# pinellolab/CRISPResso2

Measured on NVIDIA H100. Metric: reads/sec aligned+classified (250 bp, single amplicon), higher is better.
Workload: dtype int32

## Files before the change

crispresso2_b200/_lib.py:

```python
import ctypes as C
import os

import numpy as np

_HERE = os.path.dirname(os.path.abspath(__file__))
DEFAULT_LIB = os.path.join(_HERE, "libc2b200.so")

MAX_Q = 8
MAX_SEEDS = 8
MAX_READ_LEN = 512
MAX_REF_LEN = 1024
MAX_REFS = 32

F_IGNORE_SUBSTITUTIONS = 1
F_IGNORE_INSERTIONS = 2
F_IGNORE_DELETIONS = 4
F_EXPAND_AMBIGUOUS = 8
F_ASSIGN_FIRST = 16
F_DISCARD_INDEL_READS = 32
F_NO_STRAND_SEARCH = 64
F_NO_PAIRING = 128
F_HDR_REF1 = 256
F_NO_RING = 512
F_LEGACY_INS = 1024
# ... 37 lines not shown
                ("n_seeds", C.c_int32), ("tot_exon_len_mod", C.c_int32), ("coding_mask", C.c_void_p)]


ALN_DTYPE = np.dtype([("n_match", "<u2"), ("aln_len", "<u2"), ("score_milli", "<i4"), ("strand", "u1"),
                      ("status", "u1"), ("n_edits", "<u2"), ("insertion_n", "<u2"), ("deletion_n", "<u2"),
                      ("substitution_n", "<u2"), ("n_ins_all", "<u2"), ("n_ins_win", "<u2"), ("n_del_all", "<u2"),
                      ("n_del_win", "<u2"), ("n_del_pos_all", "<u2"), ("n_sub_all", "<u2"),
                      ("irregular_ends", "u1"), ("modified", "u1")])
REC_DTYPE = np.dtype([("winner_mask", "<u4"), ("best_score_milli", "<i4"), ("best_ref", "<i2"), ("n_winners", "u1"),
                      ("ambiguous", "u1"), ("status", "<u4")])
EDIT_DTYPE = np.dtype([("a", "<u2"), ("b", "<u2"), ("type", "u1"), ("in_window", "u1"), ("base", "u1"), ("pad", "u1")])
assert ALN_DTYPE.itemsize == 32 and REC_DTYPE.itemsize == 16 and EDIT_DTYPE.itemsize == 8

EXPORTS = ["c2b_create", "c2b_destroy", "c2b_last_error", "c2b_configure", "c2b_set_edit_cap", "c2b_string_width", "c2b_align_batch",
           "c2b_align_batch_compact", "c2b_ops_words", "c2b_expand_alignment", "c2b_expand_batch", "c2b_ops_device",
           "c2b_align_batch_device", "c2b_set_pair_order", "c2b_sync", "c2b_stream", "c2b_last_kernel_ms", "c2b_launch_count", "c2b_path_counts", "c2b_band_reruns", "c2b_ring_counts", "c2b_diag_counts", "c2b_route_counts", "c2b_diag_popcount_reads",
           "c2b_counts_layout", "c2b_counts_hist_layout", "c2b_counts_reset", "c2b_counts_read", "c2b_counts_device", "c2b_global_align",
           "c2b_classify_aligned", "c2b_classify_aligned_flags", "c2b_host_alloc", "c2b_host_free",
           "c2b_fastq_dedup", "c2b_fastq_dedup_buffer", "c2b_fastq_gpu_available", "c2b_fastq_dedup_gpu", "c2b_fastq_dedup_gpu_buffer", "c2b_sam_dedup_gpu_buffer", "c2b_sam_dedup_buffer", "c2b_fastq_n_reads", "c2b_fastq_n_unique", "c2b_fastq_max_len",
           "c2b_fastq_seqs", "c2b_fastq_offsets", "c2b_fastq_counts", "c2b_fastq_first_index", "c2b_fastq_free",
           "c2b_fastq_last_error", "c2b_fastq_filter", "c2b_fastq_filter_pair", "c2b_rc_merge_weights", "c2b_screen_reads", "c2b_serial_stats",
           "c2b_consensus_from_pairs", "c2b_alleles_build", "c2b_alleles_free", "c2b_alleles_n", "c2b_alleles_order", "c2b_alleles_arena", "c2b_alleles_offsets",
           "c2b_alleles_lengths", "c2b_alleles_write_tsv", "c2b_alleles_around_cut", "c2b_alleles_cut_width", "c2b_alleles_cut_fetch",
           "c2b_annotate_build", "c2b_annotate_free", "c2b_annotate_n", "c2b_annotate_arena", "c2b_annotate_offsets",
           "c2b_annotate_cigar_arena", "c2b_annotate_cigar_offsets", "c2b_annotate_flags", "c2b_annotate_mapq", "c2b_annotate_first",
           "c2b_annotate_last_record", "c2b_annotate_record_arena", "c2b_annotate_record_offsets", "c2b_annotate_write_fastq",
           "c2b_annotate_write_sam", "c2b_annotate_write_sam_passthrough"]

_cache = {}


# ... 46 lines not shown
    L.c2b_last_kernel_ms.argtypes = [vp]
    L.c2b_launch_count.restype = i64
    L.c2b_launch_count.argtypes = [vp]
    L.c2b_path_counts.restype = C.c_int
    L.c2b_path_counts.argtypes = [vp, C.POINTER(i64), C.POINTER(i64)]
    L.c2b_band_reruns.restype = i64
    L.c2b_band_reruns.argtypes = [vp]
    L.c2b_ring_counts.restype = C.c_int
    L.c2b_ring_counts.argtypes = [vp, C.POINTER(i64), C.POINTER(i64)]
    L.c2b_diag_counts.restype = C.c_int
    L.c2b_diag_counts.argtypes = [vp, C.POINTER(i64), C.POINTER(i64), C.POINTER(i64)]
    L.c2b_route_counts.restype = C.c_int
    L.c2b_route_counts.argtypes = [vp, C.POINTER(i64), C.POINTER(i64)]
    L.c2b_diag_popcount_reads.restype = C.c_int
    L.c2b_diag_popcount_reads.argtypes = [vp, C.POINTER(i64)]
    L.c2b_counts_layout.restype = C.c_int
    L.c2b_counts_layout.argtypes = [vp, C.POINTER(i32), C.POINTER(i32), C.POINTER(i32), C.POINTER(i32)]
    L.c2b_counts_hist_layout.restype = C.c_int
    L.c2b_counts_hist_layout.argtypes = [vp, C.POINTER(i32), C.POINTER(i32), C.POINTER(i32)]
    L.c2b_counts_reset.restype = C.c_int
    L.c2b_counts_reset.argtypes = [vp]
    L.c2b_counts_read.restype = C.c_int
    L.c2b_counts_read.argtypes = [vp, vp, C.c_size_t]
    L.c2b_counts_device.restype = C.c_int
    L.c2b_counts_device.argtypes = [vp, C.POINTER(vp), C.POINTER(C.c_size_t)]
    L.c2b_global_align.restype = C.c_int
    L.c2b_global_align.argtypes = [vp, C.c_char_p, i32, C.c_char_p, i32, C.c_char_p, i32, vp, vp, i32, i32,
                                   C.c_char_p, C.c_char_p, C.POINTER(i32), C.POINTER(i32)]
    L.c2b_classify_aligned.restype = C.c_int
    L.c2b_classify_aligned.argtypes = [vp, C.c_char_p, C.c_char_p, i32, C.c_char_p, i32, vp, i32, vp, vp]
# ... 84 lines not shown
```

crispresso2_b200/csrc/c2b_core.cuh:

```cuda
#pragma once
#include <stdint.h>
#include "c2b200.h"

#ifndef C2B_EMU
#include <cuda_runtime.h>
#define C2B_DEV __device__ __forceinline__
#define C2B_DEVNOINL __device__ __noinline__
namespace wp {
C2B_DEV int lane() { return threadIdx.x & 31; }
C2B_DEV int shfl_up(int v, int d) { return __shfl_up_sync(0xffffffffu, v, d); }
C2B_DEV int shfl(int v, int src) { return __shfl_sync(0xffffffffu, v, src); }
C2B_DEV uint32_t shflu(uint32_t v, int src) { return __shfl_sync(0xffffffffu, v, src); }
C2B_DEV uint32_t shflu_up(uint32_t v, int d) { return __shfl_up_sync(0xffffffffu, v, d); }
C2B_DEV int shfl_xor(int v, int m) { return __shfl_xor_sync(0xffffffffu, v, m); }
C2B_DEV uint32_t ballot(bool p) { return __ballot_sync(0xffffffffu, p); }
C2B_DEV void sync() { __syncwarp(); }
#ifdef C2B_X_INLINE_BARRIER
C2B_DEV
#else
__device__ __noinline__
#endif
void grp_sync(int g)
{
    const int w = (int)(threadIdx.x >> 5), sh = 31 - __clz(g);
// ... 72 lines not shown
    uint32_t pk_XB, pk_YB, pk_M00;
    const uint32_t *prof2;
    const uint32_t *cIe2;
    const uint32_t *g42;
    int32_t rg_ok, rg_smax, rg_gmax, rg_gsum;
    int32_t dg_ok, dg_S, dg_thr4;
    int32_t dg_c4[2 * 4 + 1];
    int32_t dg_two, dg_a4, dg_b4;
    int32_t rt_ok, rt_thr;
    int32_t rt_mx;
    int32_t rt_c[32];
    const uint4 *rt_pl;
};
constexpr int32_t RT_OFF = -(1 << 30);
constexpr int RN_DLO = 17, RN_DHI = 11;

struct WorkBlock {
    unsigned long long pair_items, single_items, band_reruns, ring_kept, ring_sent, align_settled;
    unsigned long long diag_proved, diag_listed, tier2, routed, kept;
    unsigned long long diag_popc;
    struct Launch {
        unsigned long long align_next, tier2_next, general_next;
        unsigned long long widest;
        unsigned long long left_n, tier2_n, narrow_n, diag_n;
    } launch;
};
constexpr size_t WORK_BYTES = 32 * 8;
static_assert(sizeof(WorkBlock) <= WORK_BYTES, "work block");

struct KParams {
    const uint8_t *reads; const int64_t *offsets; int64_t n_reads;
    const int32_t *count, *qweight, *ref_id;
    const int32_t *pair_order;
    c2b_read_rec *recs; c2b_aln_rec *alns; uint8_t *strings; c2b_edit *edits;
    int32_t W, edit_cap;
    const RefDev *refs; int32_t n_refs;
    int32_t out_refs, ops_refs;
    int32_t go, ge, seed_count, seed_min; uint32_t flags; int32_t nq;
    uint8_t alpha[C2B_MAX_Q]; uint8_t comp[C2B_MAX_Q];
    uint32_t *tb; int64_t tb_words_per_warp; int32_t TS;
    uint32_t *tbb; int64_t tbb_words_per_warp;
    uint32_t *tbq;
    int32_t *bnd; int64_t bnd_words_per_warp;
    uint64_t *opsbuf;
    uint64_t *rgops;
    WorkBlock *wb;
    unsigned long long *work_counter;
    uint64_t *gops; uint32_t *gmeta; int32_t NW;
    int32_t *left;
    int32_t *left2;
    int32_t *left0;
    int32_t *left1;
    int32_t route;
    const unsigned long long *n_dev;
    int32_t vstride, hstride;
    const uint32_t *stage_src;
    int32_t stage_bytes;
    const uint8_t *lut;
    int32_t phase_sync;
    const uint64_t *forced_ops;
    const int32_t *forced_n;
};

C2B_DEV int64_t oslot(const KParams &P, int64_t rd, int r) { return rd * P.out_refs + (P.ref_id ? 0 : r); }
C2B_DEV int64_t nreads(const KParams &P) { return P.n_dev ? (int64_t)*P.n_dev : P.n_reads; }

C2B_DEV const RefDev &refdev(const KParams &P, int r) { return P.refs[r]; }

// ... 1448 lines not shown
```

crispresso2_b200/csrc/c2b_engine.cu:

```cuda
#include <algorithm>
#include <atomic>
#include <mutex>
#ifndef C2B_EMU
#include <sched.h>
#include <sys/syscall.h>
#include <unistd.h>
#include <cctype>
#endif
#include <chrono>
#include <cstdio>
#include <cstdlib>
#include <cstring>
#include <string>
#include <thread>
#include <vector>

#include "c2b_core.cuh"
#include "c2b_split.cuh"
#include "c2b_annotate.cuh"
#include "c2b_fastq_int.h"

using namespace c2b;

#ifndef C2B_EMU
// ... 762 lines not shown
    const size_t tile = (size_t)e->prm.nq * e->prm.nq * r0.Ipad * 4;
    const bool can_stage = r0.pk_maxJ > 0 && !e->forced_ops;
    auto add = [&](StepKind kind, const KParams &K, int grid, int block, size_t smem) { plan.step[plan.n++] = Step{kind, K, grid, block, smem}; };
    if (split) {
        KParams A = P;
        A.left = b.left;
        if (can_stage && tile <= (size_t)e->stage_cap_a) { A.stage_bytes = (int32_t)tile; A.stage_src = r0.prof2; }
        const size_t smem_a = sizeof(ASmem) * WARPS_PER_CTA + 128 + (size_t)A.stage_bytes;
        const bool narrow = b.left2 && !P.pair_order && plan.one && !sw.no_narrow;
        if (narrow) A.left2 = b.left2;
        const bool diag = narrow && b.left0 && e->diag_any && b.n_reads >= 16 && !sw.no_diag;
        const bool route = diag && b.left1 && !sw.no_route;
        if (diag) {
            KParams D = P;
            D.left0 = b.left0;
            if (route) { D.left1 = b.left1; D.left2 = b.left2; D.route = sw.route_all ? 2 : 1; }
            const int64_t units = (b.n_reads + 31) / 32;
            add(STEP_DIAG, D, (int)std::min<int64_t>((units + D_WARPS_PER_CTA - 1) / D_WARPS_PER_CTA, (int64_t)e->grid_a * 16), D_WARPS_PER_CTA * 32, 0);
            A.pair_order = route ? b.left1 : b.left0; A.n_dev = route ? &wb->launch.narrow_n : &wb->launch.diag_n;
        }
        add(STEP_ALIGN, A, e->grid_a, WARPS_PER_CTA * 32, smem_a);
        if (narrow) {
            KParams A2 = A;
            A2.left2 = nullptr;
            A2.pair_order = b.left2; A2.n_dev = &wb->launch.tier2_n; A2.work_counter = &wb->launch.tier2_next;
            add(STEP_ALIGN, A2, e->grid_a, WARPS_PER_CTA * 32, smem_a);
        }
        KParams B = P;
        B.pair_order = diag ? b.left0 : nullptr; B.n_dev = diag ? &wb->launch.diag_n : nullptr;
        add(STEP_CLASSIFY, B, e->grid_b, B_WARPS_PER_CTA * 32, 0);
// ... 84 lines not shown
    RTCHK(rt_zero(&((WorkBlock *)e->work.p)->launch, sizeof(WorkBlock::Launch), cs));
    if (b.gmeta) RTCHK(rt_zero(b.gmeta, (size_t)b.n_reads * (b.ref_id ? 1 : e->n_refs) * 4, cs));
    if ((rc = run_plan(e, plan, cs))) return rc;
    e->launches += plan.n;
    return C2B_OK;
}

static int ensure_ops(c2b_engine *e, DevBuf &gops, DevBuf &gmeta, DevBuf &left, DevBuf &left2, DevBuf &left0, DevBuf &left1, int64_t n_reads,
                      int nr, int W)
{
    int rc;
    if ((rc = ensure(e, gops, (size_t)n_reads * nr * (W / 32) * 8))) return rc;
    if ((rc = ensure(e, gmeta, (size_t)n_reads * nr * 4))) return rc;
    if ((rc = ensure(e, left, (size_t)(n_reads + 8) * 4))) return rc;
    if ((rc = ensure(e, left2, (size_t)(n_reads + 16) * 4))) return rc;
    if ((rc = ensure(e, left0, (size_t)(n_reads + 16) * 4))) return rc;
    if ((rc = ensure(e, left1, (size_t)(n_reads + 16) * 4))) return rc;
    return C2B_OK;
}

int c2b_align_batch_device(c2b_engine *e, const uint8_t *d_reads, const int64_t *d_offsets, int64_t n_reads,
                           int32_t max_read_len, const int32_t *d_count, const int32_t *d_qweight,
                           const int32_t *d_ref_id, c2b_read_rec *d_recs, c2b_aln_rec *d_alns,
                           uint8_t *d_strings, c2b_edit *d_edits)
{
    if (!e || !e->configured) return fail(e, C2B_E_STATE, "c2b_align_batch_device: engine not configured");
#ifndef C2B_EMU
    cudaSetDevice(e->device);
#endif
    if (max_read_len < 1) max_read_len = 1;
    const int W = (e->max_I + max_read_len + 31) & ~31, nr = d_ref_id ? 1 : e->n_refs;
// ... 70 lines not shown
    if (proved) *proved = (int64_t)v.diag_proved;
    if (tier1) *tier1 = (int64_t)v.diag_listed;
    if (tier2) *tier2 = (int64_t)v.tier2;
    return C2B_OK;
}

int c2b_diag_popcount_reads(c2b_engine *e, int64_t *reads)
{
    if (!e || !e->work.p) return fail(e, C2B_E_STATE, "c2b_diag_popcount_reads: nothing launched yet");
    WorkBlock v;
    RTCHK(rt_d2h(&v, e->work.p, sizeof v, e->stream));
    RTCHK(rt_sync(e->stream));
    if (reads) *reads = (int64_t)v.diag_popc;
    return C2B_OK;
}

int c2b_route_counts(c2b_engine *e, int64_t *routed, int64_t *kept)
{
    if (!e || !e->work.p) return fail(e, C2B_E_STATE, "c2b_route_counts: nothing launched yet");
    WorkBlock v;
    RTCHK(rt_d2h(&v, e->work.p, sizeof v, e->stream));
    RTCHK(rt_sync(e->stream));
    if (routed) *routed = (int64_t)v.routed;
    if (kept) *kept = (int64_t)v.kept;
    return C2B_OK;
}

int c2b_ring_counts(c2b_engine *e, int64_t *ring_pairs, int64_t *ring_fallbacks)
{
    if (!e) return C2B_E_ARG;
// ... 616 lines not shown
```

crispresso2_b200/csrc/c2b_split.cuh:

```cuda
#pragma once
#include "c2b_core.cuh"

namespace c2b {

constexpr uint32_t GM_NONE = 0, GM_ALIGNED = 1;

C2B_DEV uint32_t gmeta_pack(int n, int strand, uint32_t state) { return (uint32_t)n | ((uint32_t)strand << 16) | (state << 24); }

struct ASmem {
    uint8_t fw[2][RG_COMBO], rc[2][RG_COMBO];
    uint8_t combo[8][RG_COMBO];
    uint32_t fin[96];
    uint8_t lut[256];
};

C2B_DEV void asmem_init(const KParams &P, ASmem &S)
{
    const int lane = wp::lane();
    for (int k = lane; k < 256; k += 32) S.lut[k] = P.lut[k];
    wp::sync();
}

C2B_DEV int64_t read_at(const KParams &P, int64_t idx) { return P.pair_order ? (int64_t)P.pair_order[idx] : idx; }

// ... 15 lines not shown
    const int lane = wp::lane();
    bool bad = false;
    for (int base = 0; base < J; base += 128) {
        uint8_t ch[4];
#pragma unroll
        for (int e = 0; e < 4; e++) { const int p = base + lane + 32 * e; ch[e] = p < J ? src[p] : (uint8_t)P.alpha[0]; }
#pragma unroll
        for (int e = 0; e < 4; e++) {
            const int p = base + lane + 32 * e;
            int code = lut[ch[e]];
            if (code == 255) { bad = true; code = 0; }
            if (p < J) { fw[p] = (uint8_t)code; rc[J - 1 - p] = P.comp[code]; }
        }
    }
    return wp::ballot(bad) != 0;
}

template <int RL = 8, int NP = 4>
C2B_DEV void walk_ring4(const KParams &P, const RefDev &R, const int *Jq, const uint2 *__restrict__ tb2, const int *s0, uint32_t mask,
                        Walked *out, const int q0 = 0)
{
    constexpr int NS = 9 * RL, B = 4 * RL;
    const int lane = wp::lane();
    const int hl = lane & 15, hb = lane & 16;
    const int TS = P.TS;
    int i[NP], j[NP], s[NP], n[NP], err[NP];
    uint32_t acc[NP], lo[NP], hi[NP];
#pragma unroll
    for (int q = 0; q < NP; q++) {
        const bool on = (mask >> q) & 1u;
// ... 92 lines not shown
            if (op == OP_NONE) continue;
            if (op == OP_M && (uint32_t)P.alpha[codes[j - 1]] == (uint32_t)R.asc[i - 1]) match++;
            i -= (op != OP_I); j -= (op != OP_J);
        }
        base_i -= tot >> 16; base_j -= tot & 0xffff;
    }
#pragma unroll
    for (int d = 8; d >= 1; d >>= 1) match += wp::shfl_xor(match, d);
    return match;
}

C2B_DEV void align_group(const KParams &P, ASmem &S, const uint32_t *staged_prof, int64_t wq, int warp_slot)
{
    const int lane = wp::lane(), g = lane >> 3;
    const int64_t first = 4 * wq;
    const bool multi = P.ref_id == nullptr && P.n_refs > 1;
    bool quad = (P.tbq != nullptr || P.tb != nullptr) && 2 * first + 7 < nreads(P) && (!multi || P.n_refs <= RG_MAX_REFS);
    int r0 = 0;
    uint32_t ringmask = 0;
    if (quad) {
        const int x = lane & 7;
        const int64_t rd = read_at(P, 2 * first + x);
        const int Jx = (int)(P.offsets[rd + 1] - P.offsets[rd]);
        const int rx = P.ref_id ? P.ref_id[rd] : 0;
        r0 = wp::shfl(rx, 0);
        const int Jn = wp::shfl_xor(Jx, 1);
        bool ok = rx == r0 && Jx == Jn && Jx >= 1 && Jx <= RG_COMBO && Jx + 32 <= P.TS;
        const int k0 = multi ? 0 : r0, k1 = multi ? P.n_refs : r0 + 1;
        for (int k = k0; k < k1; k++) {
            const RefDev &R = refdev(P, k);
            ok = ok && !R.coding && Jx <= R.pk_maxJ;
            const bool rk = P.tbq != nullptr && R.rg_ok && R.I + Jx <= PK_MAX_ALN && Jx - R.I <= RG_MAXD && R.I - Jx <= RG_MAXD;
            if (wp::ballot(rk) == 0xffffffffu) ringmask |= 1u << (k - k0);
        }
        quad = wp::ballot(ok) == 0xffffffffu;
        if (!P.tb && ringmask != (k1 - k0 >= 32 ? 0xffffffffu : (1u << (k1 - k0)) - 1u)) quad = false;
    }
    if (!quad) {
#pragma unroll 1
        for (int q = 0; q < 4; q++) {
            if (2 * (first + q) >= nreads(P)) break;
            const int64_t rdA = read_at(P, 2 * (first + q));
            if (2 * (first + q) + 1 < nreads(P)) leftover_pair(P, rdA, read_at(P, 2 * (first + q) + 1));
            else leftover_one(P, rdA);
        }
        return;
    }
    const int k0 = multi ? 0 : r0, k1 = multi ? P.n_refs : r0 + 1;
    uint2 *tbq = P.tbq ? reinterpret_cast<uint2 *>(P.tbq + (int64_t)warp_slot * P.TS * 64) : nullptr;
    uint32_t okmask = 0, modes = 0;
    uint32_t both2[RG_MAX_REFS] = {0, 0, 0, 0};
    int Jg = 0, Jmax = 0;
#pragma unroll 1
    for (int q = 0; q < 4; q++) {
        const int64_t rdA = read_at(P, 2 * (first + q)), rdB = read_at(P, 2 * (first + q) + 1);
        const int J = (int)(P.offsets[rdA + 1] - P.offsets[rdA]);
        bool bad = false;
#pragma unroll 1
        for (int x = 0; x < 2; x++) bad |= load_codes_a(P, S.lut, P.reads + P.offsets[x ? rdB : rdA], J, S.fw[x], S.rc[x]);
        wp::sync();
        int mAB = 0; bool agree = true;
        uint32_t bothq[RG_MAX_REFS] = {0, 0, 0, 0};
#pragma unroll 1
        for (int k = k0; k < k1; k++) {
            int m = 0;
#pragma unroll 1
            for (int x = 0; x < 2; x++) m |= strand_mode(P, refdev(P, k), S.fw[x], J) << (2 * x);
            if (k == k0) mAB = m;
#pragma unroll
            for (int x = 0; x < 2; x++) {
                const int mk = (m >> (2 * x)) & 3, m0 = (mAB >> (2 * x)) & 3;
                if (mk == 2) bothq[(k - k0) & (RG_MAX_REFS - 1)] |= 1u << x;
                else if (mk != (m0 == 2 ? 0 : m0)) agree = false;
            }
        }
        const int mA = mAB & 3, mB = mAB >> 2;
        if (!bad && agree) {
            const uint8_t *cA = mA == 1 ? S.rc[0] : S.fw[0], *cB = mB == 1 ? S.rc[1] : S.fw[1];
            for (int p = lane; p < J; p += 32) S.combo[q][p] = (uint8_t)(cA[p] * P.nq + cB[p]);
            okmask |= 1u << q; modes |= (uint32_t)mAB << (4 * q);
#pragma unroll
            for (int kk = 0; kk < RG_MAX_REFS; kk++) both2[kk] |= bothq[kk] << (2 * q);
            if (g == q) Jg = J;
            if (J > Jmax) Jmax = J;
        }
        wp::sync();
    }
    uint32_t good2 = 0;
#pragma unroll
    for (int q = 0; q < 4; q++) if ((okmask >> q) & 1u) good2 |= 3u << (2 * q);
    if (!P.tb) {
#pragma unroll
        for (int kk = 0; kk < RG_MAX_REFS; kk++) { good2 &= ~both2[kk]; both2[kk] = 0; }
    }
    int npass = 0, ntried = 0, nboth = 0;
#pragma unroll 1
    for (int k = k0; k < k1 && good2; k++) {
        const RefDev &R = refdev(P, k);
        const uint32_t bothk = both2[(k - k0) & (RG_MAX_REFS - 1)];
        const uint32_t ring2 = good2 & ~bothk;
        nboth += wp::popc(bothk & good2);
        const bool staged = (k == 0 && staged_prof != nullptr);
        uint32_t pass2 = 0;
        if (((ringmask >> (k - k0)) & 1u) && ring2) {
        if (staged) dp_ring<true>(P, R, staged_prof, S.combo[g], Jg, Jmax + R.lstar, tbq, S.fin);
        else dp_ring<false>(P, R, R.prof2, S.combo[g], Jg, Jmax + R.lstar, tbq, S.fin);
        wp::sync();
        const int fl = 3 * ((lane & 24) | (R.lstar & 7));
        const uint32_t cM = Jg > 0 ? S.fin[fl] : PK_SENT, cX = Jg > 0 ? S.fin[fl + 1] : PK_SENT, cY = Jg > 0 ? S.fin[fl + 2] : PK_SENT;
        wp::sync();
        const uint32_t z = wp::max3_2(cM, cY, cX);
        const uint32_t s2 = z & PK_TM;
        const int thr = ring_bound(P, R, Jg) + 512 - P.ge * (R.I + Jg);
        const bool passA = Jg > 0 && (int)((z & 0xffffu) >> 2) > thr, passB = Jg > 0 && (int)(z >> 18) > thr;
        const uint32_t bA = wp::ballot(passA), bB = wp::ballot(passB);
#pragma unroll
        for (int q = 0; q < 4; q++) pass2 |= (((bA >> (8 * q)) & 1u) | (((bB >> (8 * q)) & 1u) << 1)) << (2 * q);
        pass2 &= ring2;
        ntried += wp::popc(ring2);
        {
            int Jq[4], s0[4];
            Walked wk4[4];
            uint32_t walkmask = 0;
#pragma unroll
            for (int q = 0; q < 4; q++) {
                const uint32_t sq = wp::shflu(s2, 8 * q);
                Jq[q] = wp::shfl(Jg, 8 * q);
                s0[q] = (lane & 16) ? (int)(sq >> 16) : (int)(sq & 3u);
                if ((pass2 >> (2 * q)) & 3u) walkmask |= 1u << q;
            }
            walk_ring4(P, R, Jq, tbq, s0, walkmask, wk4);
#pragma unroll
            for (int q = 0; q < 4; q++) {
                if (!((walkmask >> q) & 1u)) continue;
                const Walked &wk = wk4[q];
                const uint32_t eb = wp::ballot(wk.err != 0);
                if (eb & 0xffffu) pass2 &= ~(1u << (2 * q));
                if (eb >> 16) pass2 &= ~(2u << (2 * q));
                const int h = lane >> 4, hl = lane & 15;
                if (!((pass2 >> (2 * q + h)) & 1u)) continue;
                const int64_t rd = read_at(P, 2 * (first + q) + h);
                const int64_t slot = oslot(P, rd, k);
                if (hl < P.NW) P.gops[slot * P.NW + hl] = wk.ops;
                if (hl == 0) {
                    const int mode = (int)((modes >> (4 * q + 2 * h)) & 3u);
                    P.gmeta[slot] = gmeta_pack(wk.n, mode == 1, GM_NONE);
                }
            }
        }
        npass += wp::popc(pass2);
        } else ntried += wp::popc(ring2);
        const uint32_t failed = ring2 & ~pass2;
        if ((failed | (bothk & good2)) && P.tb) {
            uint2 *tb2 = reinterpret_cast<uint2 *>(P.tb + (int64_t)warp_slot * P.tb_words_per_warp);
            int32_t *bnd = P.bnd + (int64_t)warp_slot * P.bnd_words_per_warp;
            const int h = lane >> 4, hl = lane & 15;
#pragma unroll 1
            for (int job = 0; job < 16; job++) {
                const int q = job >> 2, kind = job & 3;
                if (kind == 3) continue;
                const uint32_t fq = (failed >> (2 * q)) & 3u;
                const uint32_t bq = ((bothk & good2) >> (2 * q)) & 3u;
                if (kind == 0 ? fq == 0 : !((bq >> (kind - 1)) & 1u)) continue;
                const int Jp = wp::shfl(Jg, 8 * q);
                const uint8_t *combo = S.combo[q];
                wp::sync();
                if (kind) {
// ... 26 lines not shown
                    const uint32_t bit = 1u << (2 * q + kind - 1);
                    if (eb) good2 &= ~bit;
                    else if (h == pick) {
                        const int64_t rd = read_at(P, 2 * (first + q) + (kind - 1));
                        const int64_t slot = oslot(P, rd, k);
                        if (hl < P.NW) P.gops[slot * P.NW + hl] = wk.ops;
                        if (hl + 16 < P.NW) P.gops[slot * P.NW + 16 + hl] = wk.ops2;
                        if (hl == 0) P.gmeta[slot] = gmeta_pack(wk.n, pick, GM_NONE);
                    }
                }
            }
        }
        pass2 |= bothk & good2;
        good2 &= pass2;
        wp::sync();
    }
#ifndef C2B_EMU
    if (tbq && ringmask) {
        const char *base = reinterpret_cast<const char *>(tbq);
        const int64_t bytes = (int64_t)P.TS * 64 * 4;
        for (int64_t o = (int64_t)lane * 128; o < bytes; o += 32 * 128)
            asm volatile("discard.global.L2 [%0], 128;" ::"l"(base + o) : "memory");
    }
#endif
    if (lane == 0) {
        wp::addg(&P.wb->align_settled, wp::popc(good2));
        wp::addg(&P.wb->ring_kept, npass);
        wp::addg(&P.wb->ring_sent, ntried - npass + nboth + 2 * (k1 - k0) * (4 - wp::popc(okmask)));
    }
#pragma unroll 1
    for (int q = 0; q < 4; q++) {
        const int64_t rdA = read_at(P, 2 * (first + q)), rdB = read_at(P, 2 * (first + q) + 1);
        const uint32_t gq = (good2 >> (2 * q)) & 3u;
        if (gq) {
            const int64_t rd = (lane & 1) ? rdB : rdA;
            const int k = k0 + (lane >> 1);
            if (k < k1 && ((gq >> (lane & 1)) & 1u)) { const int64_t slot = oslot(P, rd, k); P.gmeta[slot] = (P.gmeta[slot] & 0x00ffffffu) | (GM_ALIGNED << 24); }
        }
        if (gq == 0) leftover_pair(P, rdA, rdB);
        else if (gq != 3u) leftover_one(P, gq == 1u ? rdB : rdA);
    }
}

C2B_DEV bool align_narrow16(const KParams &P, ASmem &S, const uint32_t *staged_prof, int64_t w16, int warp_slot)
{
    constexpr int RL = 4, DLO = 4 * RL + 1, DHI = 9 * RL - 4 * RL - 9;
    static_assert(DLO == RN_DLO && DHI == RN_DHI, "the diagonal tier's routing test assumes this band");
    const int lane = wp::lane(), g = lane >> 2;
    const int64_t first = 16 * w16;
    if (!P.left2 || P.tbq == nullptr || first + 15 >= nreads(P) || (P.ref_id == nullptr && P.n_refs > 1)) return false;
    int r0, J0;
    {
        const int64_t rd = read_at(P, first + (lane & 15));
        const int Jx = (int)(P.offsets[rd + 1] - P.offsets[rd]);
        const int rx = P.ref_id ? P.ref_id[rd] : 0;
        r0 = wp::shfl(rx, 0); J0 = wp::shfl(Jx, 0);
        const RefDev &R = refdev(P, r0);
        const bool ok = rx == r0 && Jx == J0 && Jx >= 1 && Jx <= RG_COMBO && Jx + 32 <= P.TS && R.rg_ok && !R.coding && Jx <= R.pk_maxJ &&
                        R.I + Jx <= PK_MAX_ALN && Jx - R.I <= RG_MAXD && R.I - Jx <= RG_MAXD;
        if (wp::ballot(ok) != 0xffffffffu) return false;
    }
    const RefDev &R = refdev(P, r0);
    const int J = J0;
    uint2 *tbq = reinterpret_cast<uint2 *>(P.tbq + (int64_t)warp_slot * P.TS * 64);
    uint32_t modes = 0, use2 = 0;
#pragma unroll 1
    for (int q = 0; q < 8; q++) {
        const int64_t rdA = read_at(P, first + 2 * q), rdB = read_at(P, first + 2 * q + 1);
        bool badA = load_codes_a(P, S.lut, P.reads + P.offsets[rdA], J, S.fw[0], S.rc[0]);
        bool badB = load_codes_a(P, S.lut, P.reads + P.offsets[rdB], J, S.fw[1], S.rc[1]);
        wp::sync();
        int m = 0;
#pragma unroll 1
        for (int x = 0; x < 2; x++) m |= strand_mode(P, R, S.fw[x], J) << (2 * x);
        const int mA = m & 3, mB = m >> 2;
        const uint8_t *cA = mA == 1 ? S.rc[0] : S.fw[0], *cB = mB == 1 ? S.rc[1] : S.fw[1];
        for (int p = lane; p < J; p += 32) S.combo[q][p] = (uint8_t)(cA[p] * P.nq + cB[p]);
        modes |= (uint32_t)m << (4 * q);
        if (!badA && mA != 2) use2 |= 1u << (2 * q);
        if (!badB && mB != 2) use2 |= 2u << (2 * q);
        wp::sync();
    }
    const bool staged = (r0 == 0 && staged_prof != nullptr);
    if (staged) dp_ring<true, RL>(P, R, staged_prof, S.combo[g], J, J + R.lstar, tbq, S.fin);
    else dp_ring<false, RL>(P, R, R.prof2, S.combo[g], J, J + R.lstar, tbq, S.fin);
    wp::sync();
    const int fl = 3 * ((lane & ~(RL - 1)) | (R.lstar & (RL - 1)));
    const uint32_t cM = S.fin[fl], cX = S.fin[fl + 1], cY = S.fin[fl + 2];
    wp::sync();
    const uint32_t z = wp::max3_2(cM, cY, cX);
    const uint32_t s2 = z & PK_TM;
    const int thr = ring_bound(P, R, J, DLO, DHI) + 512 - P.ge * (R.I + J);
    const uint32_t bA = wp::ballot((int)((z & 0xffffu) >> 2) > thr), bB = wp::ballot((int)(z >> 18) > thr);
    uint32_t pass2 = 0;
#pragma unroll
    for (int q = 0; q < 8; q++) pass2 |= (((bA >> (RL * q)) & 1u) | (((bB >> (RL * q)) & 1u) << 1)) << (2 * q);
    pass2 &= use2;
#pragma unroll 1
    for (int half = 0; half < 2; half++) {
        const int q0 = 4 * half;
        int Jq[4], s0[4];
        Walked wk4[4];
        uint32_t walkmask = 0;
#pragma unroll
        for (int q = 0; q < 4; q++) {
            const uint32_t sq = wp::shflu(s2, RL * (q0 + q));
            Jq[q] = J;
            s0[q] = (lane & 16) ? (int)(sq >> 16) : (int)(sq & 3u);
            if ((pass2 >> (2 * (q0 + q))) & 3u) walkmask |= 1u << q;
        }
        if (!walkmask) continue;
        walk_ring4<RL, 4>(P, R, Jq, tbq, s0, walkmask, wk4, q0);
#pragma unroll
        for (int q = 0; q < 4; q++) {
            if (!((walkmask >> q) & 1u)) continue;
            const int qq = q0 + q;
            const Walked &wk = wk4[q];
            const uint32_t eb = wp::ballot(wk.err != 0);
            if (eb & 0xffffu) pass2 &= ~(1u << (2 * qq));
            if (eb >> 16) pass2 &= ~(2u << (2 * qq));
            const int h = lane >> 4, hl = lane & 15;
            if (!((pass2 >> (2 * qq + h)) & 1u)) continue;
            const int64_t rd = read_at(P, first + 2 * qq + h);
            const int64_t slot = oslot(P, rd, r0);
            if (hl < P.NW) P.gops[slot * P.NW + hl] = wk.ops;
            if (hl == 0) P.gmeta[slot] = gmeta_pack(wk.n, (int)((modes >> (4 * qq + 2 * h)) & 3u) == 1, GM_ALIGNED);
        }
    }
#ifndef C2B_EMU
    {
        const char *base = reinterpret_cast<const char *>(tbq);
        const int64_t bytes = (int64_t)P.TS * 64 * 4;
        for (int64_t o = (int64_t)lane * 128; o < bytes; o += 32 * 128)
            asm volatile("discard.global.L2 [%0], 128;" ::"l"(base + o) : "memory");
    }
#endif
    const uint32_t rest = 0xffffu & ~pass2;
    if (lane < 16 && ((rest >> lane) & 1u)) {
        const unsigned long long pos = wp::fetch_add(&P.wb->launch.tier2_n, 1ull);
        P.left2[pos] = (int32_t)read_at(P, first + lane);
    }
    if (lane == 0) {
        wp::addg(&P.wb->align_settled, wp::popc(pass2));
        wp::addg(&P.wb->ring_kept, wp::popc(pass2));
        wp::addg(&P.wb->tier2, 16 - wp::popc(pass2));
    }
    return true;
}

C2B_DEV void align_loop(const KParams &P, ASmem &S, const uint32_t *staged_prof, int warp)
{
    const int lane = wp::lane();
    asmem_init(P, S);
    const int64_t nrd = nreads(P);
    const unsigned ahead = (unsigned)wp::grid_warps();
    if (P.left2) {
        const unsigned total = (unsigned)((nrd + 15) / 16);
        for (;;) {
            unsigned w = 0;
            if (lane == 0) w = (unsigned)wp::fetch_work(P.work_counter);
            w = (unsigned)wp::shfl((int)w, 0);
// ... 569 lines not shown
    }
    sc_flush(acc, P);
}

constexpr int DG_PROVED = 0, DG_KEEP = 1, DG_ROUTE = 2;
struct DSmem {
    uint4 pl[2][10];
    uint8_t raw[2][RG_COMBO + 32];
    int32_t pl_ref;
    uint8_t fw[RG_COMBO], rc[RG_COMBO];
    uint8_t lut[256];
    int64_t off[33];
    int64_t total_bytes;
    int32_t ref[32], cnt[32], qw[32];
    int32_t npop;
};

C2B_DEV uint32_t pl_match(uint4 a, uint4 b) { return ~((a.x ^ b.x) | (a.y ^ b.y)) & a.z & b.z; }
C2B_DEV uint4 pl_shifted(uint4 lo, uint4 hi, int t)
{
    return make_uint4(wp::funnel_r(lo.x, hi.x, t), wp::funnel_r(lo.y, hi.y, t), wp::funnel_r(lo.z, hi.z, t), 0u);
}
C2B_DEV uint32_t pl_below(int n) { return n >= 32 ? ~0u : n <= 0 ? 0u : (1u << n) - 1u; }

C2B_DEV void diag_classify(const KParams &P, const DSmem &S, const RefDev &R, const uint8_t *c, int64_t rd, int r, int strand,
                           long long cnt, long long w, ScAcc<1> &A, bool planes)
{
    const int lane = wp::lane(), I = R.I;
    const uint32_t lt = (1u << lane) - 1u;
    const int64_t slot = oslot(P, rd, r);
// ... 127 lines not shown
    const int pa = 32 * w0 + 2 * lane + 1;
    cand(pa, F0 + incl - e1);
    cand(pa + 1, F0 + incl);
    if (lane == 0) cand(32 * w0, F0);
#pragma unroll
    for (int d = 16; d >= 1; d >>= 1) { const int o = wp::shfl_xor(e, d); if (o > e) e = o; }
    return e > R.rt_thr ? DG_KEEP : DG_ROUTE;
}

C2B_DEV int diag_read(const KParams &P, DSmem &S, int64_t rd, const uint8_t *bytes, int J, int r, long long cnt, long long w,
                      ScAcc<1> &A)
{
    const int lane = wp::lane();
    const RefDev &R = refdev(P, r);
    const int I = R.I;
    if (!R.dg_ok || J != I || J > RG_COMBO || J + 32 > P.TS || J > R.pk_maxJ || I + J > PK_MAX_ALN) return DG_KEEP;
    const bool bad = load_codes_a(P, S.lut, bytes, J, S.fw, S.rc);
    wp::sync();
    if (bad) return P.route ? DG_ROUTE : DG_KEEP;
    const int mode = strand_mode(P, R, S.fw, J);
    if (mode == 2) return P.route ? DG_ROUTE : DG_KEEP;
    const uint8_t *c = mode == 1 ? S.rc : S.fw;
    const int nb = (I + 31) >> 5, dS = R.dg_S;
    uint4 rp = make_uint4(0u, 0u, 0u, 0u);
    bool acgt = false;
    if (R.dg_two || R.rt_ok) {
        for (int b = 0; b < nb; b++) {
            const int x = 32 * b + lane, q = x < I ? c[x] : 255;
            const uint32_t p0 = wp::ballot(q & 1), p1 = wp::ballot(q & 2), v = wp::ballot(q < 4);
            if (lane == b) rp = make_uint4(p0, p1, v, 0u);
        }
        acgt = wp::ballot(lane < nb && rp.z != pl_below(I - 32 * lane)) == 0;
        if (lane < nb + 2) S.pl[0][lane] = rp;
        const bool fresh = S.pl_ref != r;
        wp::sync();
// ... 113 lines not shown
#endif
    uint32_t fail = 0, route = 0;
    diag_stage(P, S, 0, 0);
#pragma unroll 1
    for (int x = 0; x < n; x++) {
        const int64_t off = S.off[x];
        wp::wait_async();
        wp::sync();
        if (x + 1 < n) diag_stage(P, S, x + 1, (x + 1) & 1);
        const int v = diag_read(P, S, first + x, S.raw[x & 1] + ((uintptr_t)(P.reads + off) & 15), (int)(S.off[x + 1] - off), S.ref[x],
                                S.cnt[x], S.qw[x], A);
        if (v != DG_PROVED) fail |= 1u << x;
        if (v == DG_ROUTE) route |= 1u << x;
        wp::sync();
    }
    list_append(P.left0, &P.wb->launch.diag_n, fail, first);
    if (P.route) {
        list_append(P.left1, &P.wb->launch.narrow_n, fail & ~route, first);
        list_append(P.left2, &P.wb->launch.tier2_n, route, first);
    }
    routed = wp::popc(route);
    return n - wp::popc(fail);
}

C2B_DEV void diag_loop(const KParams &P, DSmem &S, int64_t warp, int64_t nwarps)
{
    dsmem_init(P, S);
    ScAcc<1> acc;
    sc_init(acc);
    const int64_t units = (P.n_reads + 31) / 32;
// ... 20 lines not shown
```

crispresso2_b200/engine.py:

```python
import ctypes as C

import numpy as np

from . import _lib

_DNA_COMP = {"A": "T", "C": "G", "G": "C", "T": "A"}


class EngineError(RuntimeError):
    pass


class BatchResult:

    def __init__(self, recs, alns, strings, edits, W, ops=None, meta=None, engine=None, buf=None, off=None, ref_id=None):
        self.recs, self.alns, self.strings, self.edits, self.W = recs, alns, strings, edits, W
        self.ops, self.meta, self._engine, self._buf, self._off, self._ref_id = ops, meta, engine, buf, off, ref_id

    def strings_block(self, lo, hi):
        if self.strings is not None:
            return self.strings[lo:hi]
        e = self._engine
        off = np.ascontiguousarray(self._off[lo:hi + 1])
        rid = None if self._ref_id is None else np.ascontiguousarray(self._ref_id[lo:hi], dtype=np.int32)
# ... 228 lines not shown
    def diag_counts(self):
        a, b, c = C.c_int64(0), C.c_int64(0), C.c_int64(0)
        self._check(self.L.c2b_diag_counts(self.h, C.byref(a), C.byref(b), C.byref(c)), "c2b_diag_counts")
        return a.value, b.value, c.value

    def route_counts(self):
        a, b = C.c_int64(0), C.c_int64(0)
        self._check(self.L.c2b_route_counts(self.h, C.byref(a), C.byref(b)), "c2b_route_counts")
        return a.value, b.value

    def diag_popcount_reads(self):
        a = C.c_int64(0)
        self._check(self.L.c2b_diag_popcount_reads(self.h, C.byref(a)), "c2b_diag_popcount_reads")
        return a.value

    def launch_count(self):
        return int(self.L.c2b_launch_count(self.h))
```

include/c2b200.h:

```cpp
#ifndef C2B200_H
#define C2B200_H
#include <stddef.h>
#include <stdint.h>

#ifdef __cplusplus
extern "C" {
#endif

#define C2B_MAX_Q        8
#define C2B_MAX_SEEDS    8
#define C2B_MAX_SEED_LEN 20
#define C2B_MAX_REF_LEN  1024
#define C2B_MAX_READ_LEN 512
#define C2B_MAX_ALN_LEN  1024
#define C2B_MAX_REFS     32
#define C2B_MAX_POOLED_REFS 1024

#define C2B_OK            0
#define C2B_E_CUDA       -1
#define C2B_E_ARG        -2
#define C2B_E_LIMIT      -3
#define C2B_E_STATE      -4

#define C2B_F_IGNORE_SUBSTITUTIONS  1u
// ... 137 lines not shown
                            int32_t max_read_len, const int32_t *d_count, const int32_t *d_qweight,
                            const int32_t *d_ref_id, c2b_read_rec *d_recs, c2b_aln_rec *d_alns,
                            uint8_t *d_strings, c2b_edit *d_edits);
int  c2b_set_pair_order(c2b_engine *e, const int32_t *d_order);
int  c2b_ops_device(c2b_engine *e, void **d_ops, void **d_meta);
int  c2b_sync(c2b_engine *e);
void *c2b_stream(c2b_engine *e);
double c2b_last_kernel_ms(c2b_engine *e);
int64_t c2b_launch_count(const c2b_engine *e);
int  c2b_path_counts(c2b_engine *e, int64_t *pair_items, int64_t *single_items);
int64_t c2b_band_reruns(c2b_engine *e);
int  c2b_ring_counts(c2b_engine *e, int64_t *ring_pairs, int64_t *ring_fallbacks);
int  c2b_diag_counts(c2b_engine *e, int64_t *proved, int64_t *tier1, int64_t *tier2);
int  c2b_route_counts(c2b_engine *e, int64_t *routed, int64_t *kept);
int  c2b_diag_popcount_reads(c2b_engine *e, int64_t *reads);

int  c2b_counts_layout(const c2b_engine *e, int32_t *n_refs, int32_t *n_vec, int32_t *stride, int32_t *n_scal);
int  c2b_counts_hist_layout(const c2b_engine *e, int32_t *n_hist, int32_t *hstride, int32_t *hist_zero);
int  c2b_counts_reset(c2b_engine *e);
int  c2b_counts_read(c2b_engine *e, int64_t *out, size_t n_int64);
int  c2b_counts_device(c2b_engine *e, void **d_ptr, size_t *n_int64);

int  c2b_global_align(c2b_engine *e, const char *read, int32_t read_len, const char *ref, int32_t ref_len,
                      const char *alphabet, int32_t nq, const int64_t *score_rows, const int64_t *gap_incentive,
                      int32_t gap_open, int32_t gap_extend,
                      char *out_read, char *out_ref, int32_t *aln_len, int32_t *n_match);

int  c2b_classify_aligned(c2b_engine *e, const char *read_al, const char *ref_al, int32_t n_cols,
                          const char *alphabet, int32_t nq, const int64_t *include_idx, int32_t n_include,
                          c2b_aln_rec *out, c2b_edit *edits);
// ... 102 lines not shown
```

Baseline: 88.85 million.

## Cache diagonal-tier strand-seed results per read and reuse them in align tiers

The diagonal tier now records, per read, whether the strand/seed test ran, its mode, and whether the read had bad bases, in a byte array placed after left0. The narrow and quad align tiers read these bytes and skip reloading codes and rerunning strand_mode when both reads of a pair were already tested; the narrow tier builds the combo row straight from raw bytes. The L2 discard of traceback scratch is removed, and optional clock64 phase counters plus a seed-test counter are added. The cost is an extra byte buffer, additional global reads, and one atomic per remaining strand_mode call.

```diff
diff --git a/crispresso2_b200/_lib.py b/crispresso2_b200/_lib.py
--- a/crispresso2_b200/_lib.py
+++ b/crispresso2_b200/_lib.py
@@ -75,7 +75,7 @@
 
 EXPORTS = ["c2b_create", "c2b_destroy", "c2b_last_error", "c2b_configure", "c2b_set_edit_cap", "c2b_string_width", "c2b_align_batch",
            "c2b_align_batch_compact", "c2b_ops_words", "c2b_expand_alignment", "c2b_expand_batch", "c2b_ops_device",
-           "c2b_align_batch_device", "c2b_set_pair_order", "c2b_sync", "c2b_stream", "c2b_last_kernel_ms", "c2b_launch_count", "c2b_path_counts", "c2b_band_reruns", "c2b_ring_counts", "c2b_diag_counts", "c2b_route_counts", "c2b_diag_popcount_reads",
+           "c2b_align_batch_device", "c2b_set_pair_order", "c2b_sync", "c2b_stream", "c2b_last_kernel_ms", "c2b_launch_count", "c2b_path_counts", "c2b_band_reruns", "c2b_ring_counts", "c2b_diag_counts", "c2b_route_counts", "c2b_diag_popcount_reads", "c2b_align_seed_tests",
            "c2b_counts_layout", "c2b_counts_hist_layout", "c2b_counts_reset", "c2b_counts_read", "c2b_counts_device", "c2b_global_align",
            "c2b_classify_aligned", "c2b_classify_aligned_flags", "c2b_host_alloc", "c2b_host_free",
            "c2b_fastq_dedup", "c2b_fastq_dedup_buffer", "c2b_fastq_gpu_available", "c2b_fastq_dedup_gpu", "c2b_fastq_dedup_gpu_buffer", "c2b_sam_dedup_gpu_buffer", "c2b_sam_dedup_buffer", "c2b_fastq_n_reads", "c2b_fastq_n_unique", "c2b_fastq_max_len",
@@ -152,6 +152,8 @@
     L.c2b_route_counts.argtypes = [vp, C.POINTER(i64), C.POINTER(i64)]
     L.c2b_diag_popcount_reads.restype = C.c_int
     L.c2b_diag_popcount_reads.argtypes = [vp, C.POINTER(i64)]
+    L.c2b_align_seed_tests.restype = C.c_int
+    L.c2b_align_seed_tests.argtypes = [vp, C.POINTER(i64)]
     L.c2b_counts_layout.restype = C.c_int
     L.c2b_counts_layout.argtypes = [vp, C.POINTER(i32), C.POINTER(i32), C.POINTER(i32), C.POINTER(i32)]
     L.c2b_counts_hist_layout.restype = C.c_int
diff --git a/crispresso2_b200/csrc/c2b_core.cuh b/crispresso2_b200/csrc/c2b_core.cuh
--- a/crispresso2_b200/csrc/c2b_core.cuh
+++ b/crispresso2_b200/csrc/c2b_core.cuh
@@ -110,11 +110,13 @@
 };
 constexpr int32_t RT_OFF = -(1 << 30);
 constexpr int RN_DLO = 17, RN_DHI = 11;
+constexpr int SEED_TESTED = 0x80, SEED_BAD = 0x04;
 
 struct WorkBlock {
     unsigned long long pair_items, single_items, band_reruns, ring_kept, ring_sent, align_settled;
     unsigned long long diag_proved, diag_listed, tier2, routed, kept;
     unsigned long long diag_popc;
+    unsigned long long align_seed;
     struct Launch {
         unsigned long long align_next, tier2_next, general_next;
         unsigned long long widest;
@@ -123,6 +125,17 @@
 };
 constexpr size_t WORK_BYTES = 32 * 8;
 static_assert(sizeof(WorkBlock) <= WORK_BYTES, "work block");
+
+enum { APH_PROLOGUE, APH_DP, APH_BOUND, APH_WALK, APH_EPILOGUE, APH_FULL, APH_N };
+#if defined(C2B_ALIGN_PHASES) && !defined(C2B_EMU)
+__device__ unsigned long long c2b_aph[2][APH_N];
+#define C2B_APH_START(t) long long t = clock64()
+#define C2B_APH_LAP(t, tier, ph) do { const long long t_ = clock64(); \
+        if (wp::lane() == 0) atomicAdd(&c2b_aph[tier][ph], (unsigned long long)(t_ - (t))); (t) = t_; } while (0)
+#else
+#define C2B_APH_START(t) do {} while (0)
+#define C2B_APH_LAP(t, tier, ph) do {} while (0)
+#endif
 
 struct KParams {
     const uint8_t *reads; const int64_t *offsets; int64_t n_reads;
@@ -148,6 +161,7 @@
     int32_t *left0;
     int32_t *left1;
     int32_t route;
+    uint8_t *seedb;
     const unsigned long long *n_dev;
     int32_t vstride, hstride;
     const uint32_t *stage_src;
diff --git a/crispresso2_b200/csrc/c2b_engine.cu b/crispresso2_b200/csrc/c2b_engine.cu
--- a/crispresso2_b200/csrc/c2b_engine.cu
+++ b/crispresso2_b200/csrc/c2b_engine.cu
@@ -800,6 +800,7 @@
         if (diag) {
             KParams D = P;
             D.left0 = b.left0;
+            D.seedb = A.seedb = reinterpret_cast<uint8_t *>(b.left0 + b.n_reads + 16);
             if (route) { D.left1 = b.left1; D.left2 = b.left2; D.route = sw.route_all ? 2 : 1; }
             const int64_t units = (b.n_reads + 31) / 32;
             add(STEP_DIAG, D, (int)std::min<int64_t>((units + D_WARPS_PER_CTA - 1) / D_WARPS_PER_CTA, (int64_t)e->grid_a * 16), D_WARPS_PER_CTA * 32, 0);
@@ -914,7 +915,7 @@
     if ((rc = ensure(e, gmeta, (size_t)n_reads * nr * 4))) return rc;
     if ((rc = ensure(e, left, (size_t)(n_reads + 8) * 4))) return rc;
     if ((rc = ensure(e, left2, (size_t)(n_reads + 16) * 4))) return rc;
-    if ((rc = ensure(e, left0, (size_t)(n_reads + 16) * 4))) return rc;
+    if ((rc = ensure(e, left0, (size_t)(n_reads + 16) * 5))) return rc;
     if ((rc = ensure(e, left1, (size_t)(n_reads + 16) * 4))) return rc;
     return C2B_OK;
 }
@@ -1015,6 +1016,26 @@
     if (reads) *reads = (int64_t)v.diag_popc;
     return C2B_OK;
 }
+
+int c2b_align_seed_tests(c2b_engine *e, int64_t *calls)
+{
+    if (!e || !e->work.p) return fail(e, C2B_E_STATE, "c2b_align_seed_tests: nothing launched yet");
+    WorkBlock v;
+    RTCHK(rt_d2h(&v, e->work.p, sizeof v, e->stream));
+    RTCHK(rt_sync(e->stream));
+    if (calls) *calls = (int64_t)v.align_seed;
+    return C2B_OK;
+}
+
+#if defined(C2B_ALIGN_PHASES) && !defined(C2B_EMU)
+extern "C" int c2b_align_phase_cycles(c2b_engine *e, unsigned long long *out)
+{
+    if (!e) return C2B_E_ARG;
+    if (cudaDeviceSynchronize() != cudaSuccess || cudaMemcpyFromSymbol(out, c2b_aph, sizeof c2b_aph) != cudaSuccess) return C2B_E_STATE;
+    static const unsigned long long zero[2][APH_N] = {};
+    return cudaMemcpyToSymbol(c2b_aph, zero, sizeof zero) == cudaSuccess ? C2B_OK : C2B_E_STATE;
+}
+#endif
 
 int c2b_route_counts(c2b_engine *e, int64_t *routed, int64_t *kept)
 {
diff --git a/crispresso2_b200/csrc/c2b_split.cuh b/crispresso2_b200/csrc/c2b_split.cuh
--- a/crispresso2_b200/csrc/c2b_split.cuh
+++ b/crispresso2_b200/csrc/c2b_split.cuh
@@ -53,6 +53,36 @@
         }
     }
     return wp::ballot(bad) != 0;
+}
+
+C2B_DEV int align_strand_mode(const KParams &P, const RefDev &R, const uint8_t *fw, int J)
+{
+    if (wp::lane() == 0) wp::addg(&P.wb->align_seed, 1);
+    return strand_mode(P, R, fw, J);
+}
+
+C2B_DEV void combo_row(const KParams &P, const uint8_t *lut, uint8_t *dst, const uint8_t *a, const uint8_t *b, int J, bool ra, bool rb)
+{
+    const int lane = wp::lane();
+    for (int base = 0; base < J; base += 128) {
+        uint8_t ca[4], cb[4];
+#pragma unroll
+        for (int e = 0; e < 4; e++) {
+            const int p = base + lane + 32 * e;
+            if (p < J) { ca[e] = a[ra ? J - 1 - p : p]; cb[e] = b[rb ? J - 1 - p : p]; }
+        }
+#pragma unroll
+        for (int e = 0; e < 4; e++) {
+            const int p = base + lane + 32 * e;
+            if (p >= J) break;
+            int u = lut[ca[e]], v = lut[cb[e]];
+            if (u == 255) u = 0;
+            if (v == 255) v = 0;
+            if (ra) u = P.comp[u];
+            if (rb) v = P.comp[v];
+            dst[p] = (uint8_t)(u * P.nq + v);
+        }
+    }
 }
 
 template <int RL = 8, int NP = 4>
@@ -175,6 +205,7 @@
 {
     const int lane = wp::lane(), g = lane >> 3;
     const int64_t first = 4 * wq;
+    C2B_APH_START(tph);
     const bool multi = P.ref_id == nullptr && P.n_refs > 1;
     bool quad = (P.tbq != nullptr || P.tb != nullptr) && 2 * first + 7 < nreads(P) && (!multi || P.n_refs <= RG_MAX_REFS);
     int r0 = 0;
@@ -205,6 +236,7 @@
             if (2 * (first + q) + 1 < nreads(P)) leftover_pair(P, rdA, read_at(P, 2 * (first + q) + 1));
             else leftover_one(P, rdA);
         }
+        C2B_APH_LAP(tph, 1, APH_EPILOGUE);
         return;
     }
     const int k0 = multi ? 0 : r0, k1 = multi ? P.n_refs : r0 + 1;
@@ -216,6 +248,8 @@
     for (int q = 0; q < 4; q++) {
         const int64_t rdA = read_at(P, 2 * (first + q)), rdB = read_at(P, 2 * (first + q) + 1);
         const int J = (int)(P.offsets[rdA + 1] - P.offsets[rdA]);
+        const int sAB = (P.seedb && k1 - k0 == 1) ? (P.seedb[rdA] | (P.seedb[rdB] << 8)) : 0;
+        const bool reuse = (sAB & (SEED_TESTED | (SEED_TESTED << 8))) == (SEED_TESTED | (SEED_TESTED << 8));
         bool bad = false;
 #pragma unroll 1
         for (int x = 0; x < 2; x++) bad |= load_codes_a(P, S.lut, P.reads + P.offsets[x ? rdB : rdA], J, S.fw[x], S.rc[x]);
@@ -225,8 +259,11 @@
 #pragma unroll 1
         for (int k = k0; k < k1; k++) {
             int m = 0;
-#pragma unroll 1
-            for (int x = 0; x < 2; x++) m |= strand_mode(P, refdev(P, k), S.fw[x], J) << (2 * x);
+            if (reuse) m = (sAB & 3) | ((sAB >> 6) & 12);
+            else {
+#pragma unroll 1
+                for (int x = 0; x < 2; x++) m |= align_strand_mode(P, refdev(P, k), S.fw[x], J) << (2 * x);
+            }
             if (k == k0) mAB = m;
 #pragma unroll
             for (int x = 0; x < 2; x++) {
@@ -250,6 +287,7 @@
     uint32_t good2 = 0;
 #pragma unroll
     for (int q = 0; q < 4; q++) if ((okmask >> q) & 1u) good2 |= 3u << (2 * q);
+    C2B_APH_LAP(tph, 1, APH_PROLOGUE);
     if (!P.tb) {
 #pragma unroll
         for (int kk = 0; kk < RG_MAX_REFS; kk++) { good2 &= ~both2[kk]; both2[kk] = 0; }
@@ -264,9 +302,11 @@
         const bool staged = (k == 0 && staged_prof != nullptr);
         uint32_t pass2 = 0;
         if (((ringmask >> (k - k0)) & 1u) && ring2) {
+        C2B_APH_LAP(tph, 1, APH_EPILOGUE);
         if (staged) dp_ring<true>(P, R, staged_prof, S.combo[g], Jg, Jmax + R.lstar, tbq, S.fin);
         else dp_ring<false>(P, R, R.prof2, S.combo[g], Jg, Jmax + R.lstar, tbq, S.fin);
         wp::sync();
+        C2B_APH_LAP(tph, 1, APH_DP);
         const int fl = 3 * ((lane & 24) | (R.lstar & 7));
         const uint32_t cM = Jg > 0 ? S.fin[fl] : PK_SENT, cX = Jg > 0 ? S.fin[fl + 1] : PK_SENT, cY = Jg > 0 ? S.fin[fl + 2] : PK_SENT;
         wp::sync();
@@ -279,6 +319,7 @@
         for (int q = 0; q < 4; q++) pass2 |= (((bA >> (8 * q)) & 1u) | (((bB >> (8 * q)) & 1u) << 1)) << (2 * q);
         pass2 &= ring2;
         ntried += wp::popc(ring2);
+        C2B_APH_LAP(tph, 1, APH_BOUND);
         {
             int Jq[4], s0[4];
             Walked wk4[4];
@@ -291,6 +332,7 @@
                 if ((pass2 >> (2 * q)) & 3u) walkmask |= 1u << q;
             }
             walk_ring4(P, R, Jq, tbq, s0, walkmask, wk4);
+            C2B_APH_LAP(tph, 1, APH_WALK);
 #pragma unroll
             for (int q = 0; q < 4; q++) {
                 if (!((walkmask >> q) & 1u)) continue;
@@ -312,6 +354,7 @@
         npass += wp::popc(pass2);
         } else ntried += wp::popc(ring2);
         const uint32_t failed = ring2 & ~pass2;
+        C2B_APH_LAP(tph, 1, APH_EPILOGUE);
         if ((failed | (bothk & good2)) && P.tb) {
             uint2 *tb2 = reinterpret_cast<uint2 *>(P.tb + (int64_t)warp_slot * P.tb_words_per_warp);
             int32_t *bnd = P.bnd + (int64_t)warp_slot * P.bnd_words_per_warp;
@@ -368,15 +411,8 @@
         pass2 |= bothk & good2;
         good2 &= pass2;
         wp::sync();
-    }
-#ifndef C2B_EMU
-    if (tbq && ringmask) {
-        const char *base = reinterpret_cast<const char *>(tbq);
-        const int64_t bytes = (int64_t)P.TS * 64 * 4;
-        for (int64_t o = (int64_t)lane * 128; o < bytes; o += 32 * 128)
-            asm volatile("discard.global.L2 [%0], 128;" ::"l"(base + o) : "memory");
-    }
-#endif
+        C2B_APH_LAP(tph, 1, APH_FULL);
+    }
     if (lane == 0) {
         wp::addg(&P.wb->align_settled, wp::popc(good2));
         wp::addg(&P.wb->ring_kept, npass);
@@ -394,6 +430,7 @@
         if (gq == 0) leftover_pair(P, rdA, rdB);
         else if (gq != 3u) leftover_one(P, gq == 1u ? rdB : rdA);
     }
+    C2B_APH_LAP(tph, 1, APH_EPILOGUE);
 }
 
 C2B_DEV bool align_narrow16(const KParams &P, ASmem &S, const uint32_t *staged_prof, int64_t w16, int warp_slot)
@@ -402,6 +439,7 @@
     static_assert(DLO == RN_DLO && DHI == RN_DHI, "the diagonal tier's routing test assumes this band");
     const int lane = wp::lane(), g = lane >> 2;
     const int64_t first = 16 * w16;
+    C2B_APH_START(tph);
     if (!P.left2 || P.tbq == nullptr || first + 15 >= nreads(P) || (P.ref_id == nullptr && P.n_refs > 1)) return false;
     int r0, J0;
     {
@@ -421,24 +459,37 @@
 #pragma unroll 1
     for (int q = 0; q < 8; q++) {
         const int64_t rdA = read_at(P, first + 2 * q), rdB = read_at(P, first + 2 * q + 1);
-        bool badA = load_codes_a(P, S.lut, P.reads + P.offsets[rdA], J, S.fw[0], S.rc[0]);
-        bool badB = load_codes_a(P, S.lut, P.reads + P.offsets[rdB], J, S.fw[1], S.rc[1]);
-        wp::sync();
-        int m = 0;
-#pragma unroll 1
-        for (int x = 0; x < 2; x++) m |= strand_mode(P, R, S.fw[x], J) << (2 * x);
+        const uint8_t *a = P.reads + P.offsets[rdA], *b = P.reads + P.offsets[rdB];
+        const int sAB = P.seedb ? (P.seedb[rdA] | (P.seedb[rdB] << 8)) : 0;
+        const bool reuse = (sAB & (SEED_TESTED | (SEED_TESTED << 8))) == (SEED_TESTED | (SEED_TESTED << 8));
+        int m = 0, bad;
+        if (reuse) {
+            m = (sAB & 3) | ((sAB >> 6) & 12);
+            bad = ((sAB & SEED_BAD) ? 1 : 0) | ((sAB & (SEED_BAD << 8)) ? 2 : 0);
+        } else {
+            bad = (load_codes_a(P, S.lut, a, J, S.fw[0], S.rc[0]) ? 1 : 0) | (load_codes_a(P, S.lut, b, J, S.fw[1], S.rc[1]) ? 2 : 0);
+            wp::sync();
+#pragma unroll 1
+            for (int x = 0; x < 2; x++) m |= align_strand_mode(P, R, S.fw[x], J) << (2 * x);
+        }
         const int mA = m & 3, mB = m >> 2;
-        const uint8_t *cA = mA == 1 ? S.rc[0] : S.fw[0], *cB = mB == 1 ? S.rc[1] : S.fw[1];
-        for (int p = lane; p < J; p += 32) S.combo[q][p] = (uint8_t)(cA[p] * P.nq + cB[p]);
+        if (reuse) combo_row(P, S.lut, S.combo[q], a, b, J, mA == 1, mB == 1);
+        else {
+            const uint8_t *cA = mA == 1 ? S.rc[0] : S.fw[0], *cB = mB == 1 ? S.rc[1] : S.fw[1];
+            for (int p = lane; p < J; p += 32) S.combo[q][p] = (uint8_t)(cA[p] * P.nq + cB[p]);
+            wp::sync();
+        }
         modes |= (uint32_t)m << (4 * q);
-        if (!badA && mA != 2) use2 |= 1u << (2 * q);
-        if (!badB && mB != 2) use2 |= 2u << (2 * q);
-        wp::sync();
-    }
+        if (!(bad & 1) && mA != 2) use2 |= 1u << (2 * q);
+        if (!(bad & 2) && mB != 2) use2 |= 2u << (2 * q);
+    }
+    wp::sync();
     const bool staged = (r0 == 0 && staged_prof != nullptr);
+    C2B_APH_LAP(tph, 0, APH_PROLOGUE);
     if (staged) dp_ring<true, RL>(P, R, staged_prof, S.combo[g], J, J + R.lstar, tbq, S.fin);
     else dp_ring<false, RL>(P, R, R.prof2, S.combo[g], J, J + R.lstar, tbq, S.fin);
     wp::sync();
+    C2B_APH_LAP(tph, 0, APH_DP);
     const int fl = 3 * ((lane & ~(RL - 1)) | (R.lstar & (RL - 1)));
     const uint32_t cM = S.fin[fl], cX = S.fin[fl + 1], cY = S.fin[fl + 2];
     wp::sync();
@@ -450,6 +501,7 @@
 #pragma unroll
     for (int q = 0; q < 8; q++) pass2 |= (((bA >> (RL * q)) & 1u) | (((bB >> (RL * q)) & 1u) << 1)) << (2 * q);
     pass2 &= use2;
+    C2B_APH_LAP(tph, 0, APH_BOUND);
 #pragma unroll 1
     for (int half = 0; half < 2; half++) {
         const int q0 = 4 * half;
@@ -464,7 +516,9 @@
             if ((pass2 >> (2 * (q0 + q))) & 3u) walkmask |= 1u << q;
         }
         if (!walkmask) continue;
+        C2B_APH_LAP(tph, 0, APH_EPILOGUE);
         walk_ring4<RL, 4>(P, R, Jq, tbq, s0, walkmask, wk4, q0);
+        C2B_APH_LAP(tph, 0, APH_WALK);
 #pragma unroll
         for (int q = 0; q < 4; q++) {
             if (!((walkmask >> q) & 1u)) continue;
@@ -481,14 +535,6 @@
             if (hl == 0) P.gmeta[slot] = gmeta_pack(wk.n, (int)((modes >> (4 * qq + 2 * h)) & 3u) == 1, GM_ALIGNED);
         }
     }
-#ifndef C2B_EMU
-    {
-        const char *base = reinterpret_cast<const char *>(tbq);
-        const int64_t bytes = (int64_t)P.TS * 64 * 4;
-        for (int64_t o = (int64_t)lane * 128; o < bytes; o += 32 * 128)
-            asm volatile("discard.global.L2 [%0], 128;" ::"l"(base + o) : "memory");
-    }
-#endif
     const uint32_t rest = 0xffffu & ~pass2;
     if (lane < 16 && ((rest >> lane) & 1u)) {
         const unsigned long long pos = wp::fetch_add(&P.wb->launch.tier2_n, 1ull);
@@ -499,6 +545,7 @@
         wp::addg(&P.wb->ring_kept, wp::popc(pass2));
         wp::addg(&P.wb->tier2, 16 - wp::popc(pass2));
     }
+    C2B_APH_LAP(tph, 0, APH_EPILOGUE);
     return true;
 }
 
@@ -1098,6 +1145,7 @@
     int64_t total_bytes;
     int32_t ref[32], cnt[32], qw[32];
     int32_t npop;
+    uint8_t seed[32];
 };
 
 C2B_DEV uint32_t pl_match(uint4 a, uint4 b) { return ~((a.x ^ b.x) | (a.y ^ b.y)) & a.z & b.z; }
@@ -1255,11 +1303,19 @@
     const int lane = wp::lane();
     const RefDev &R = refdev(P, r);
     const int I = R.I;
-    if (!R.dg_ok || J != I || J > RG_COMBO || J + 32 > P.TS || J > R.pk_maxJ || I + J > PK_MAX_ALN) return DG_KEEP;
+    uint8_t *seed = lane == 0 ? S.seed + (rd & 31) : nullptr;
+    if (!R.dg_ok || J != I || J > RG_COMBO || J + 32 > P.TS || J > R.pk_maxJ || I + J > PK_MAX_ALN) {
+        if (seed) *seed = 0;
+        return DG_KEEP;
+    }
     const bool bad = load_codes_a(P, S.lut, bytes, J, S.fw, S.rc);
     wp::sync();
-    if (bad) return P.route ? DG_ROUTE : DG_KEEP;
+    if (bad) {
+        if (seed) *seed = SEED_TESTED | SEED_BAD;
+        return P.route ? DG_ROUTE : DG_KEEP;
+    }
     const int mode = strand_mode(P, R, S.fw, J);
+    if (seed) *seed = (uint8_t)(SEED_TESTED | mode);
     if (mode == 2) return P.route ? DG_ROUTE : DG_KEEP;
     const uint8_t *c = mode == 1 ? S.rc : S.fw;
     const int nb = (I + 31) >> 5, dS = R.dg_S;
@@ -1403,6 +1459,7 @@
         if (v == DG_ROUTE) route |= 1u << x;
         wp::sync();
     }
+    if (P.seedb && lane < n) P.seedb[first + lane] = S.seed[lane];
     list_append(P.left0, &P.wb->launch.diag_n, fail, first);
     if (P.route) {
         list_append(P.left1, &P.wb->launch.narrow_n, fail & ~route, first);
diff --git a/crispresso2_b200/engine.py b/crispresso2_b200/engine.py
--- a/crispresso2_b200/engine.py
+++ b/crispresso2_b200/engine.py
@@ -266,5 +266,10 @@
         self._check(self.L.c2b_diag_popcount_reads(self.h, C.byref(a)), "c2b_diag_popcount_reads")
         return a.value
 
+    def align_seed_tests(self):
+        a = C.c_int64(0)
+        self._check(self.L.c2b_align_seed_tests(self.h, C.byref(a)), "c2b_align_seed_tests")
+        return a.value
+
     def launch_count(self):
         return int(self.L.c2b_launch_count(self.h))
diff --git a/include/c2b200.h b/include/c2b200.h
--- a/include/c2b200.h
+++ b/include/c2b200.h
@@ -175,6 +175,7 @@
 int  c2b_diag_counts(c2b_engine *e, int64_t *proved, int64_t *tier1, int64_t *tier2);
 int  c2b_route_counts(c2b_engine *e, int64_t *routed, int64_t *kept);
 int  c2b_diag_popcount_reads(c2b_engine *e, int64_t *reads);
+int  c2b_align_seed_tests(c2b_engine *e, int64_t *calls);
 
 int  c2b_counts_layout(const c2b_engine *e, int32_t *n_refs, int32_t *n_vec, int32_t *stride, int32_t *n_scal);
 int  c2b_counts_hist_layout(const c2b_engine *e, int32_t *n_hist, int32_t *hstride, int32_t *hist_zero);
```

Result: faster. 90.41 million, median of 6 (+1.8%).
